# ZhangLearning/llm-message-queue

Hardware: AMD Instinct MI355X
Metric: requests/sec + p99 enqueue->dispatch latency, 4-tier mix at 1/2/4/8 backends (higher is better)
Workload: dtype bf16

## Files before the change

csrc/kernels/gemm_kernels.h:

```cpp
#pragma once

#include <hip/hip_runtime.h>
#include <stdint.h>

#include <type_traits>

#include "fp8_decode.h"
#include "sample_noise.h"

namespace llmq {

typedef __attribute__((ext_vector_type(8))) short gm_bf16x8;
typedef __attribute__((ext_vector_type(4))) float gm_f32x4;
typedef __attribute__((ext_vector_type(4))) unsigned int gm_u32x4;

constexpr int GM_BM = 256, GM_BN = 256, GM_BK = 64, GM_THREADS = 512;
constexpr int GM_HALF_BYTES = 128 * GM_BK * 2;
constexpr int GM_BUF_BYTES = 4 * GM_HALF_BYTES;
constexpr int GM_LDS_BYTES = 2 * GM_BUF_BYTES;
constexpr int GM_GROUP_M = 8;

enum { GM_EPI_STORE = 0, GM_EPI_SWIGLU = 2, GM_EPI_ROPE = 3, GM_EPI_ARGMAX = 4, GM_EPI_RESID = 5,
       GM_EPI_RESID_LDS = 6, GM_EPI_RESID_PRE = 7, GM_EPI_RESID_RMS = 8, GM_EPI_SAMPLE = 9 };
constexpr int GM_LDS_SPARE = 32768;
template <int EPI>
constexpr int gm_lds_bytes() { return EPI == GM_EPI_RESID_PRE ? GM_LDS_BYTES + GM_LDS_SPARE : GM_LDS_BYTES; }

enum {
  GM_DIAG_NONE = 0,
  GM_DIAG_SKIP_A2 = 1,
  GM_DIAG_NO_LDS_READ = 2,
  GM_DIAG_NO_DMA = 3,
  GM_DIAG_CLOCK = 4,
  GM_DIAG_CLOCK_NO_DMA = 5,
  GM_DIAG_L2_PANELS = 6
};

struct GmSide {
  float* pv;
  int32_t* pi;
  union {
    float* rpart;
    const float* inv_temp;
  };
  union {
    int* rticket;
    const uint32_t* key;
  };
  float* rscale;
  float reps;
};

struct GmRope {
  const int32_t* pos;
  const int32_t* slot;
  const float* cos_t;
  const float* sin_t;
  uint16_t* q;
  uint16_t* kc;
  uint16_t* vc;
  int Hq, Hkv, max_ctx, n_slots;
};
enum { GM_A0 = 0, GM_A1 = 1, GM_B0 = 2, GM_B1 = 3 };

__device__ __forceinline__ uint16_t gm_f2bf(float f) {
  uint32_t u = __float_as_uint(f);
  u += 0x7fffu + ((u >> 16) & 1u);
  return (uint16_t)(u >> 16);
}

__device__ __forceinline__ void gm_load_row_scales(const float* __restrict__ rs, int row0, int fq,
                                                   gm_f32x4 (&sc)[2][4]) {
  if (rs) {
#pragma unroll
    for (int mh = 0; mh < 2; ++mh)
#pragma unroll
      for (int m = 0; m < 4; ++m)
        sc[mh][m] = *reinterpret_cast<const gm_f32x4*>(rs + row0 + mh * 64 + m * 16 + fq * 4);
  } else {
#pragma unroll
    for (int mh = 0; mh < 2; ++mh)
#pragma unroll
      for (int m = 0; m < 4; ++m) sc[mh][m] = gm_f32x4{1.f, 1.f, 1.f, 1.f};
  }
}

#define GM_CPOL_SC1 16

struct GmSplit {
  int full;
  float* ws;
  int* cnt;
};

typedef __attribute__((address_space(3))) void* gm_lds_ptr;
typedef gm_f32x4 gm_acc_t[2][4][2][2];

__device__ __forceinline__ void gm_stage(__amdgpu_buffer_rsrc_t rs, uint32_t v0, uint32_t v1, uint32_t soff,
                                         uint8_t* smem, uint32_t dst0, uint32_t dst1) {
  __builtin_amdgcn_raw_ptr_buffer_load_lds(rs, (gm_lds_ptr)(smem + dst0), 16, v0, soff, 0, 0);
  __builtin_amdgcn_raw_ptr_buffer_load_lds(rs, (gm_lds_ptr)(smem + dst1), 16, v1, soff, 0, 0);
}

#define GM_LGKM(N) asm volatile("s_waitcnt lgkmcnt(" #N ")" ::: "memory")
#define GM_VMCNT(N) asm volatile("s_waitcnt vmcnt(%0)" ::"n"(N) : "memory")
#define GM_FENCE() __builtin_amdgcn_sched_barrier(0)
#define GM_BARRIER()                  \
  do {                                \
    GM_FENCE();                       \
    __builtin_amdgcn_s_barrier();     \
    GM_FENCE();                       \
  } while (0)

typedef __attribute__((ext_vector_type(2))) unsigned int gf_u32x2;
template <int OFF>
__device__ __forceinline__ gf_u32x2 gf_lds_read_b64(uint32_t addr) {
  gf_u32x2 r;
  asm volatile("ds_read_b64 %0, %1 offset:%2" : "=v"(r) : "v"(addr), "n"(OFF) : "memory");
  return r;
}

template <int PER>
__device__ __forceinline__ int gm_xcd_run_start(int b, int count) {
  const int n = PER * count;
  const int xcd = b & 7, q8 = n >> 3, r8 = n & 7;
  return xcd < r8 ? xcd * (q8 + 1) : r8 * (q8 + 1) + (xcd - r8) * q8;
}

struct GmTile {
  int tm, tn;
  int pid;
  int khalf;
};

__device__ __forceinline__ GmTile gm_tile_coords(int bid, int tiles_m, int tiles_n, int nwg, int full,
                                                 int group_m) {
  GmTile t;
  t.khalf = -1;
  if (bid < full) {
    t.pid = gm_xcd_run_start<1>(bid, full) + (bid >> 3);
  } else {
    const int b = bid - full;
    const int j = gm_xcd_run_start<2>(b, nwg - full) + (b >> 3);
    t.pid = full + (j >> 1);
    t.khalf = j & 1;
  }
  const int group = t.pid / (group_m * tiles_n);
  const int first_m = group * group_m;
  const int gsize = min(tiles_m - first_m, group_m);
  t.tm = first_m + (t.pid % (group_m * tiles_n)) % gsize;
  t.tn = (t.pid % (group_m * tiles_n)) / gsize;
  return t;
}

__device__ __forceinline__ bool gm_split_join(uint8_t* __restrict__ smem, gm_acc_t& acc, const GmSplit& sp,
                                              int tix) {
  const int tid = threadIdx.x;
  int* cnt = sp.cnt + 2 * tix;
  if (tid == 0) *reinterpret_cast<int*>(smem) =
      __hip_atomic_fetch_add(cnt, 1, __ATOMIC_RELAXED, __HIP_MEMORY_SCOPE_AGENT);
  __syncthreads();
  const int ticket = *reinterpret_cast<volatile int*>(smem);
  __syncthreads();
  float* slab = sp.ws + (size_t)tix * GM_THREADS * 128;
  const __amdgpu_buffer_rsrc_t srs = __builtin_amdgcn_make_buffer_rsrc(slab, 0, GM_THREADS * 32 * 16, 0x00020000);
  if (ticket == 0) {
#pragma unroll
    for (int a = 0; a < 2; ++a)
#pragma unroll
      for (int b = 0; b < 4; ++b)
#pragma unroll
        for (int c = 0; c < 2; ++c)
#pragma unroll
          for (int d = 0; d < 2; ++d)
          {
            const int i = ((a * 4 + b) * 4 + c * 2 + d) * GM_THREADS + tid;
            __builtin_amdgcn_raw_buffer_store_b128(__builtin_bit_cast(gm_u32x4, acc[a][b][c][d]), srs, i * 16,
                                                   0, GM_CPOL_SC1);
          }
    GM_VMCNT(0);
    __syncthreads();
    if (tid == 0) __hip_atomic_store(cnt + 1, 1, __ATOMIC_RELAXED, __HIP_MEMORY_SCOPE_AGENT);
    return true;
  }
  if (tid == 0) {
    for (int spin = 0; spin < (1 << 24); ++spin) {
      if (__hip_atomic_load(cnt + 1, __ATOMIC_RELAXED, __HIP_MEMORY_SCOPE_AGENT)) break;
      __builtin_amdgcn_s_sleep(2);
    }
    GM_VMCNT(0);
    __hip_atomic_store(cnt, 0, __ATOMIC_RELAXED, __HIP_MEMORY_SCOPE_AGENT);
    __hip_atomic_store(cnt + 1, 0, __ATOMIC_RELAXED, __HIP_MEMORY_SCOPE_AGENT);
  }
  __syncthreads();
#pragma unroll
  for (int a = 0; a < 2; ++a)
#pragma unroll
    for (int b = 0; b < 4; ++b)
#pragma unroll
      for (int c = 0; c < 2; ++c)
#pragma unroll
        for (int d = 0; d < 2; ++d)
        {
          const int i = ((a * 4 + b) * 4 + c * 2 + d) * GM_THREADS + tid;
          acc[a][b][c][d] += __builtin_bit_cast(gm_f32x4, __builtin_amdgcn_raw_buffer_load_b128(
                                 srs, i * 16, 0, GM_CPOL_SC1));
        }
  return false;
}


template <int EPI, int DIAG, bool FP8 = false>
__device__ __forceinline__ void gemm_tile(
    uint8_t* __restrict__ smem, const uint16_t* __restrict__ A, const void* __restrict__ W,
    const float* __restrict__ cs, uint16_t* __restrict__ C, int M, int N, int K, int group_m,
    const float* __restrict__ rs, const GmRope& rp, const GmSplit& sp, const GmSide& am, const int bid) {
  static_assert(!FP8 || (DIAG == GM_DIAG_NONE &&
                         (EPI == GM_EPI_STORE || EPI == GM_EPI_SWIGLU || EPI == GM_EPI_RESID_LDS)),
                "the FP8 form: STORE, SWIGLU and RESID_LDS, no diagnostics");
  constexpr int kBHalf = 128 * GM_BK * (FP8 ? 1 : 2);
  constexpr int kBuf = 2 * GM_HALF_BYTES + 2 * kBHalf;
  static_assert(2 * kBuf <= GM_LDS_BYTES, "operand buffers inside the launch's LDS");
  constexpr bool kStamp = DIAG == GM_DIAG_CLOCK || DIAG == GM_DIAG_CLOCK_NO_DMA;
  const int tiles_m = (M + GM_BM - 1) / GM_BM;
  const int tiles_n = N / GM_BN;
  const int nwg = tiles_m * tiles_n;
  const int full = sp.ws ? sp.full : nwg;
  const GmTile tile = gm_tile_coords(bid, tiles_m, tiles_n, nwg, full, group_m);
  const int pid = tile.pid, khalf = tile.khalf, tm = tile.tm, tn = tile.tn;

  const int tid = threadIdx.x;
  const int lane = tid & 63;
  const int w = __builtin_amdgcn_readfirstlane(tid >> 6);
  uint64_t st_t0 = 0, st_r0 = 0;
  if constexpr (kStamp) {
    st_t0 = __builtin_amdgcn_s_memtime();
    st_r0 = __builtin_amdgcn_s_memrealtime();
  }
  const int wr = w >> 2, wc = w & 3;

  const int srow = w * 8 + (lane >> 3);
  const int schunk = (lane & 7) ^ ((srow >> 1) & 7);
  const int brow = w * 16 + (lane >> 2);
  const int bchunk = (lane & 3) ^ ((brow >> 2) & 3);
  const __amdgpu_buffer_rsrc_t rsa = __builtin_amdgcn_make_buffer_rsrc((void*)A, 0, M * K * 2, 0x00020000);
  const __amdgpu_buffer_rsrc_t rsw =
      __builtin_amdgcn_make_buffer_rsrc((void*)W, 0, N * K * (FP8 ? 1 : 2), 0x00020000);
  uint32_t va[2][2], vb[2][FP8 ? 1 : 2];
  const int ltm = DIAG == GM_DIAG_L2_PANELS ? 0 : tm, ltn = DIAG == GM_DIAG_L2_PANELS ? 0 : tn;
#pragma unroll
  for (int h = 0; h < 2; ++h) {
#pragma unroll
    for (int i = 0; i < 2; ++i) {
      int row = ltm * GM_BM + i * 128 + h * 64 + srow;
      row = row < M ? row : M - 1;
      va[h][i] = (uint32_t)row * (uint32_t)K * 2u + (uint32_t)schunk * 16u;
      if constexpr (!FP8) {
        const int col = ltn * GM_BN + (2 * i + (w >> 2)) * 64 + h * 32 + (w & 3) * 8 + (lane >> 3);
        vb[h][i] = (uint32_t)col * (uint32_t)K * 2u + (uint32_t)schunk * 16u;
      }
    }
    if constexpr (FP8) {
      const int col = ltn * GM_BN + (brow >> 5) * 64 + h * 32 + (brow & 31);
      vb[h][0] = (uint32_t)col * (uint32_t)K + (uint32_t)bchunk * 16u;
    }
  }
  const uint32_t dst_i0 = (uint32_t)(w * 8) * 128u;
  const uint32_t dst_i1 = (uint32_t)(64 + w * 8) * 128u;
  const uint32_t dst_b = (uint32_t)(w * 16) * 64u;

  const uint32_t sbase = (uint32_t)(uintptr_t)(__attribute__((address_space(3))) uint8_t*)smem;
  const int fr = lane & 15, fq = lane >> 4;
  uint32_t aoff[2][2], boff[2][2];
#pragma unroll
  for (int kk = 0; kk < 2; ++kk) {
    const int c = fq + 4 * kk;
    aoff[0][kk] = (uint32_t)(wr * 64 + fr) * 128u + (uint32_t)((c ^ ((fr >> 1) & 7)) * 16);
    if constexpr (FP8)
      boff[0][kk] = (uint32_t)(2 * GM_HALF_BYTES) + (uint32_t)(wc * 32 + fr) * 64u +
                    (uint32_t)(((c >> 1) ^ ((fr >> 2) & 3)) * 16 + (c & 1) * 8);
    else
      boff[0][kk] = (uint32_t)(wc * 32 + fr) * 128u + (uint32_t)((c ^ ((fr >> 1) & 7)) * 16) + 2 * GM_HALF_BYTES;
    aoff[1][kk] = aoff[0][kk] + kBuf;
    boff[1][kk] = boff[0][kk] + kBuf;
  }

  gm_acc_t acc;
#pragma unroll
  for (int a = 0; a < 2; ++a)
#pragma unroll
    for (int b = 0; b < 4; ++b)
#pragma unroll
      for (int c = 0; c < 2; ++c)
#pragma unroll
        for (int d = 0; d < 2; ++d) acc[a][b][c][d] = gm_f32x4{0.f, 0.f, 0.f, 0.f};

  gm_bf16x8 af[4][2];
  using gm_bfrag = std::conditional_t<FP8, gf_u32x2, gm_bf16x8>;
  gm_bfrag bfr[2][2][2];
  gm_bfrag b0y[2][2];
  const int nt = khalf < 0 ? K / GM_BK : K / GM_BK / 2;
  const int kt0 = khalf > 0 ? nt : 0;

#define GM_STAGE(BUF, HALF, KT)                                                               \
  do {                                                                                        \
    if constexpr (FP8 && (HALF) >= 2) {                                                       \
      __builtin_amdgcn_raw_ptr_buffer_load_lds(                                               \
          rsw, (gm_lds_ptr)(smem + (uint32_t)(BUF) * kBuf + 2 * GM_HALF_BYTES + (uint32_t)((HALF)-2) * kBHalf + dst_b), \
          16, vb[(HALF)-2][0], (uint32_t)((KT) + kt0) * GM_BK, 0, 0);                         \
    } else {                                                                                  \
      const uint32_t _ko = (uint32_t)((KT) + kt0) * (GM_BK * 2);                              \
      const uint32_t _b = (uint32_t)(BUF) * kBuf + (uint32_t)(HALF) * GM_HALF_BYTES;          \
      if constexpr ((HALF) < 2)                                                               \
        gm_stage(rsa, va[(HALF)][0], va[(HALF)][1], _ko, smem, _b + dst_i0, _b + dst_i1);     \
      else                                                                                    \
        gm_stage(rsw, vb[(HALF)-2][0], vb[(HALF)-2][1], _ko, smem, _b + dst_i0, _b + dst_i1); \
    }                                                                                         \
  } while (0)

#define GM_READ_A(BUF, MH)                                                                     \
  do {                                                                                         \
    _Pragma("unroll") for (int m = 0; m < 4; ++m)                                              \
      _Pragma("unroll") for (int kk = 0; kk < 2; ++kk)                                         \
        af[m][kk] = *reinterpret_cast<const gm_bf16x8*>(smem + aoff[BUF][kk] + (MH) * GM_HALF_BYTES + m * 2048); \
  } while (0)

#define GM_READ_B_INTO(BUF, NH, DST)                                                           \
  do {                                                                                         \
    if constexpr (FP8) {                                                                       \
      _Pragma("unroll") for (int kk = 0; kk < 2; ++kk) {                                       \
        DST[0][kk] = gf_lds_read_b64<(NH) * kBHalf>(sbase + boff[BUF][kk]);                    \
        DST[1][kk] = gf_lds_read_b64<(NH) * kBHalf + 1024>(sbase + boff[BUF][kk]);             \
      }                                                                                        \
    } else {                                                                                   \
      _Pragma("unroll") for (int n = 0; n < 2; ++n)                                            \
        _Pragma("unroll") for (int kk = 0; kk < 2; ++kk)                                       \
          DST[n][kk] = *reinterpret_cast<const gm_bf16x8*>(smem + boff[BUF][kk] + (NH) * kBHalf + n * 2048); \
    }                                                                                          \
  } while (0)
#define GM_READ_B(BUF, NH) GM_READ_B_INTO(BUF, NH, bfr[NH])
#define GM_READ_B0_INTO(BUF, DST) GM_READ_B_INTO(BUF, 0, DST)

#define GM_MFMA_WITH(MH, NH, BREG)                                                             \
  do {                                                                                         \
    _Pragma("unroll") for (int kk = 0; kk < 2; ++kk) {                                         \
      gm_bf16x8 _b[2];                                                                         \
      _Pragma("unroll") for (int n = 0; n < 2; ++n) {                                          \
        if constexpr (FP8) _b[n] = sk_fp8x8_bf16(BREG[n][kk].x, BREG[n][kk].y);                \
        else _b[n] = BREG[n][kk];                                                              \
      }                                                                                        \
      _Pragma("unroll") for (int m = 0; m < 4; ++m)                                            \
        _Pragma("unroll") for (int n = 0; n < 2; ++n)                                          \
          acc[MH][m][NH][n] = __builtin_amdgcn_mfma_f32_16x16x32_bf16(af[m][kk], _b[n],        \
                                                                      acc[MH][m][NH][n], 0, 0, 0); \
    }                                                                                          \
  } while (0)

#define GM_PHASE_END(MH, NH, BREG)   \
  do {                               \
    GM_BARRIER();                    \
    GM_LGKM(0);                      \
    if constexpr (FP8) GM_FENCE();   \
    GM_MFMA_WITH(MH, NH, BREG);      \
    GM_BARRIER();                    \
  } while (0)

  constexpr int kDmaA = 2, kDmaB = FP8 ? 1 : 2;
  constexpr int kFlyA = 2 * kDmaA + kDmaB, kFlyB = kDmaA + 2 * kDmaB;

  if (wr == 1) __builtin_amdgcn_s_setprio(1);
  if constexpr (EPI == GM_EPI_RESID_PRE) {
    const int col0p = tn * GM_BN + wc * 64, row0p = tm * GM_BM + wr * 128;
    const __amdgpu_buffer_rsrc_t rsp =
        __builtin_amdgcn_make_buffer_rsrc((void*)C, 0, (uint32_t)M * (uint32_t)N * 2u, 0x00020000);
#pragma unroll
    for (int i = 0; i < 4; ++i) {
      const int r = i * 8 + (lane >> 3), c = lane & 7;
      const uint32_t vo = ((uint32_t)(row0p + r) * (uint32_t)N + (uint32_t)(col0p + c * 8)) * 2u;
      __builtin_amdgcn_raw_ptr_buffer_load_lds(rsp, (gm_lds_ptr)(smem + GM_LDS_BYTES + w * 4096 + i * 1024), 16,
                                               vo, 0, 0, 0);
    }
  }
  GM_STAGE(0, GM_B0, 0);
  GM_STAGE(0, GM_A0, 0);
  GM_STAGE(0, GM_B1, 0);
  GM_STAGE(0, GM_A1, 0);
  GM_STAGE(1, GM_B0, 1);
  GM_STAGE(1, GM_A0, 1);
  GM_STAGE(1, GM_B1, 1);
  GM_VMCNT(kFlyB);
  GM_BARRIER();
  GM_READ_B0_INTO(0, bfr[0]);
  if constexpr (DIAG >= GM_DIAG_SKIP_A2 && DIAG <= GM_DIAG_NO_DMA) {
    GM_READ_A(0, 0);
    GM_READ_B(0, 1);
    GM_READ_B0_INTO(1, b0y);
  }
  if (wr == 1) GM_BARRIER();

  int t = 0;
  constexpr bool kRdA = DIAG != GM_DIAG_NO_LDS_READ;
  constexpr bool kRdA2 = DIAG != GM_DIAG_SKIP_A2 && DIAG != GM_DIAG_NO_LDS_READ;
  constexpr bool kRdB = DIAG != GM_DIAG_NO_LDS_READ;
  constexpr bool kDma = DIAG != GM_DIAG_NO_DMA && DIAG != GM_DIAG_CLOCK_NO_DMA;
#define GM_D_READ_A(ON, B, H) do { if constexpr (ON) GM_READ_A(B, H); } while (0)
#define GM_D_READ_B(B, H) do { if constexpr (kRdB) GM_READ_B(B, H); } while (0)
#define GM_D_READ_B0(B, D) do { if constexpr (kRdB) GM_READ_B0_INTO(B, D); } while (0)
#define GM_D_STAGE(B, H, K) do { if constexpr (kDma) GM_STAGE(B, H, K); } while (0)
  for (; t < nt - 2; t += 2) {
    {
      GM_D_READ_A(kRdA, 0, 0); GM_D_STAGE(1, GM_A1, t + 1); GM_VMCNT(kFlyA); GM_PHASE_END(0, 0, bfr[0]);
      GM_D_READ_B(0, 1); GM_D_STAGE(0, GM_B0, t + 2); GM_VMCNT(kFlyB); GM_PHASE_END(0, 1, bfr[1]);
      GM_D_READ_A(kRdA2, 0, 1); GM_D_STAGE(0, GM_A0, t + 2); GM_VMCNT(kFlyA); GM_PHASE_END(1, 1, bfr[1]);
      GM_D_READ_B0(1, b0y); GM_D_STAGE(0, GM_B1, t + 2); GM_VMCNT(kFlyB); GM_PHASE_END(1, 0, bfr[0]);
      GM_D_READ_A(kRdA, 1, 0); GM_D_STAGE(0, GM_A1, t + 2); GM_VMCNT(kFlyA); GM_PHASE_END(0, 0, b0y);
      GM_D_READ_B(1, 1); GM_D_STAGE(1, GM_B0, t + 3); GM_VMCNT(kFlyB); GM_PHASE_END(0, 1, bfr[1]);
      GM_D_READ_A(kRdA2, 1, 1); GM_D_STAGE(1, GM_A0, t + 3); GM_VMCNT(kFlyA); GM_PHASE_END(1, 1, bfr[1]);
      GM_D_READ_B0(0, bfr[0]); GM_D_STAGE(1, GM_B1, t + 3); GM_VMCNT(kFlyB); GM_PHASE_END(1, 0, b0y);
    }
  }
  {
      GM_READ_A(0, 0); GM_STAGE(1, GM_A1, t + 1); GM_VMCNT(kFlyA); GM_PHASE_END(0, 0, bfr[0]);
      GM_READ_B(0, 1); GM_VMCNT(kDmaA + kDmaB); GM_PHASE_END(0, 1, bfr[1]);
      GM_READ_A(0, 1); GM_VMCNT(kDmaA); GM_PHASE_END(1, 1, bfr[1]);
      GM_READ_B0_INTO(1, b0y); GM_VMCNT(0); GM_PHASE_END(1, 0, bfr[0]);
      GM_READ_A(1, 0); GM_PHASE_END(0, 0, b0y);
      GM_READ_B(1, 1); GM_PHASE_END(0, 1, bfr[1]);
      GM_READ_A(1, 1); GM_PHASE_END(1, 1, bfr[1]);
      GM_PHASE_END(1, 0, b0y);
  }
  __builtin_amdgcn_s_setprio(0);
  if (wr == 0) GM_BARRIER();
#undef GM_D_READ_A
#undef GM_D_READ_B
#undef GM_D_READ_B0
#undef GM_D_STAGE
#undef GM_PHASE_END
#undef GM_MFMA_WITH
#undef GM_READ_B0_INTO
#undef GM_READ_B
#undef GM_READ_B_INTO
#undef GM_READ_A
#undef GM_STAGE

  if (khalf >= 0 && gm_split_join(smem, acc, sp, pid - full)) return;

  if constexpr (FP8) {
    const float* csp = cs + tn * GM_BN + wc * 64 + fr;
#pragma unroll
    for (int nh = 0; nh < 2; ++nh)
#pragma unroll
      for (int n = 0; n < 2; ++n) {
        const float s = csp[nh * 32 + n * 16];
#pragma unroll
        for (int mh = 0; mh < 2; ++mh)
#pragma unroll
          for (int m = 0; m < 4; ++m) acc[mh][m][nh][n] *= s;
      }
  }

  const int row0 = tm * GM_BM + wr * 128;
  if constexpr (EPI == GM_EPI_ARGMAX || EPI == GM_EPI_SAMPLE) {
    if constexpr (EPI == GM_EPI_SAMPLE) {
      const uint32_t col = (uint32_t)(tn * GM_BN + wc * 64 + fr);
#pragma unroll
      for (int mh = 0; mh < 2; ++mh)
#pragma unroll
        for (int m = 0; m < 4; ++m) {
          const int r4 = row0 + mh * 64 + m * 16 + fq * 4;
          const gm_f32x4 it = *reinterpret_cast<const gm_f32x4*>(am.inv_temp + r4);
          const gm_u32x4 ka = *reinterpret_cast<const gm_u32x4*>(am.key + 2 * r4);
          const gm_u32x4 kb = *reinterpret_cast<const gm_u32x4*>(am.key + 2 * r4 + 4);
#pragma unroll
          for (int j = 0; j < 4; ++j) {
            const uint32_t k0 = j < 2 ? ka[2 * j] : kb[2 * j - 4];
            const uint32_t k1 = j < 2 ? ka[2 * j + 1] : kb[2 * j - 3];
            if (it[j] != 0.f) {
#pragma unroll
              for (int nh = 0; nh < 2; ++nh)
#pragma unroll
                for (int n = 0; n < 2; ++n)
                  acc[mh][m][nh][n][j] = acc[mh][m][nh][n][j] * it[j] + sn_gumbel(k0, k1, col + nh * 32 + n * 16);
            }
          }
        }
    }
    float* lv = reinterpret_cast<float*>(smem);
    int* lc = reinterpret_cast<int*>(smem + GM_BM * 4 * 4);
#pragma unroll
    for (int mh = 0; mh < 2; ++mh)
#pragma unroll
      for (int m = 0; m < 4; ++m)
#pragma unroll
        for (int j = 0; j < 4; ++j) {
          float v = acc[mh][m][0][0][j];
          int c = fr;
#pragma unroll
          for (int nh = 0; nh < 2; ++nh)
#pragma unroll
            for (int n = 0; n < 2; ++n) {
              const float x = acc[mh][m][nh][n][j];
              if (x > v) { v = x; c = nh * 32 + n * 16 + fr; }
            }
#pragma unroll
          for (int off = 1; off < 16; off <<= 1) {
            const float ov = __shfl_xor(v, off, 64);
            const int oc = __shfl_xor(c, off, 64);
            if (ov > v || (ov == v && oc < c)) { v = ov; c = oc; }
          }
          if (fr == 0) {
            const int r = wr * 128 + mh * 64 + m * 16 + fq * 4 + j;
            lv[r * 4 + wc] = v;
            lc[r * 4 + wc] = wc * 64 + c;
          }
        }
    __syncthreads();
    if (tid < GM_BM) {
      const int grow = tm * GM_BM + tid;
      float v = lv[tid * 4];
      int c = lc[tid * 4];
#pragma unroll
      for (int k = 1; k < 4; ++k)
        if (lv[tid * 4 + k] > v) { v = lv[tid * 4 + k]; c = lc[tid * 4 + k]; }
      if (grow < M) {
        am.pv[(int64_t)grow * tiles_n + tn] = v;
        am.pi[(int64_t)grow * tiles_n + tn] = tn * GM_BN + c;
      }
    }
  } else if constexpr (EPI == GM_EPI_RESID) {
    float* o = reinterpret_cast<float*>(smem + w * (32 * 68 * 4));
    const int col0 = tn * GM_BN + wc * 64;
    uint2 cres[2][2][8];
#pragma unroll
    for (int mh = 0; mh < 2; ++mh)
#pragma unroll
      for (int mp = 0; mp < 2; ++mp)
#pragma unroll
        for (int it = 0; it < 8; ++it) {
          const int qd = it * 64 + lane;
          const int grow = row0 + mh * 64 + mp * 32 + (qd >> 4);
          cres[mh][mp][it] = grow < M ? *reinterpret_cast<const uint2*>(C + (int64_t)grow * N + col0 + (qd & 15) * 4)
                                      : make_uint2(0u, 0u);
        }
#pragma unroll
    for (int mh = 0; mh < 2; ++mh)
#pragma unroll
      for (int mp = 0; mp < 2; ++mp) {
#pragma unroll
        for (int mm = 0; mm < 2; ++mm)
#pragma unroll
          for (int nh = 0; nh < 2; ++nh)
#pragma unroll
            for (int n = 0; n < 2; ++n)
#pragma unroll
              for (int j = 0; j < 4; ++j)
                o[(mm * 16 + fq * 4 + j) * 68 + nh * 32 + n * 16 + fr] = acc[mh][mp * 2 + mm][nh][n][j];
        GM_LGKM(0);
        __builtin_amdgcn_wave_barrier();
#pragma unroll
        for (int it = 0; it < 8; ++it) {
          const int qd = it * 64 + lane;
          const int r = qd >> 4, c4 = qd & 15;
          const int grow = row0 + mh * 64 + mp * 32 + r;
          const gm_f32x4 v = *reinterpret_cast<const gm_f32x4*>(o + r * 68 + c4 * 4);
          if (grow < M) {
            uint2* cp = reinterpret_cast<uint2*>(C + (int64_t)grow * N + col0 + c4 * 4);
            const uint2 cr = cres[mh][mp][it];
            const float r0 = __uint_as_float(cr.x << 16) + v[0], r1 = __uint_as_float(cr.x & 0xffff0000u) + v[1];
            const float r2 = __uint_as_float(cr.y << 16) + v[2], r3 = __uint_as_float(cr.y & 0xffff0000u) + v[3];
            *cp = make_uint2((uint32_t)gm_f2bf(r0) | ((uint32_t)gm_f2bf(r1) << 16),
                             (uint32_t)gm_f2bf(r2) | ((uint32_t)gm_f2bf(r3) << 16));
          }
        }
        GM_LGKM(0);
        __builtin_amdgcn_wave_barrier();
      }
  } else if constexpr (EPI == GM_EPI_RESID_LDS || EPI == GM_EPI_RESID_PRE || EPI == GM_EPI_RESID_RMS) {
    constexpr int kPre = EPI == GM_EPI_RESID_PRE ? 4 : 0;
    uint8_t* cw = smem + w * 16384;
    uint8_t* cpre = smem + GM_LDS_BYTES + w * 4096;
    auto rowp = [&](int r) -> uint8_t* { return (kPre && r < 32) ? cpre + r * 128 : cw + r * 128; };
    const int col0 = tn * GM_BN + wc * 64;
    const __amdgpu_buffer_rsrc_t rsc =
        __builtin_amdgcn_make_buffer_rsrc((void*)C, 0, (uint32_t)M * (uint32_t)N * 2u, 0x00020000);
#pragma unroll
    for (int i = kPre; i < 16; ++i) {
      const int r = i * 8 + (lane >> 3), c = lane & 7;
      const uint32_t vo = ((uint32_t)(row0 + r) * (uint32_t)N + (uint32_t)(col0 + c * 8)) * 2u;
      __builtin_amdgcn_raw_ptr_buffer_load_lds(rsc, (gm_lds_ptr)(cw + i * 1024), 16, vo, 0, 0, 0);
    }
    GM_VMCNT(0);
    __builtin_amdgcn_wave_barrier();
#pragma unroll
    for (int mh = 0; mh < 2; ++mh)
#pragma unroll
      for (int m = 0; m < 4; ++m)
#pragma unroll
        for (int nh = 0; nh < 2; ++nh)
#pragma unroll
          for (int n = 0; n < 2; ++n)
#pragma unroll
            for (int j = 0; j < 4; ++j) {
              const int r = mh * 64 + m * 16 + fq * 4 + j;
              uint16_t* e = reinterpret_cast<uint16_t*>(rowp(r) + (nh * 32 + n * 16 + fr) * 2);
              *e = gm_f2bf(__uint_as_float((uint32_t)*e << 16) + acc[mh][m][nh][n][j]);
            }
    GM_LGKM(0);
    __builtin_amdgcn_wave_barrier();
    constexpr bool rms = EPI == GM_EPI_RESID_RMS;
    float ssq[16];
#pragma unroll
    for (int it = 0; it < 16; ++it) {
      const int qd = it * 64 + lane;
      const int r = qd >> 3, cb = qd & 7;
      const int grow = row0 + r;
      const gm_u32x4 v = *reinterpret_cast<const gm_u32x4*>(rowp(r) + cb * 16);
      if (grow < M) *reinterpret_cast<gm_u32x4*>(C + (int64_t)grow * N + col0 + cb * 8) = v;
      if constexpr (rms) {
        float q = 0.f;
#pragma unroll
        for (int e = 0; e < 4; ++e) {
          const float lo = __uint_as_float(v[e] << 16), hi = __uint_as_float(v[e] & 0xFFFF0000u);
          q += lo * lo + hi * hi;
        }
        ssq[it] = q;
      }
    }
    if constexpr (rms) {
#pragma unroll
      for (int it = 0; it < 16; ++it) {
        float q = ssq[it];
        q += __shfl_xor(q, 1, 64);
        q += __shfl_xor(q, 2, 64);
        q += __shfl_xor(q, 4, 64);
        ssq[it] = q;
      }
      GM_LGKM(0);
      __builtin_amdgcn_wave_barrier();
      float* wp = reinterpret_cast<float*>(cw);
      if ((lane & 7) == 0) {
#pragma unroll
        for (int it = 0; it < 16; ++it) wp[it * 8 + (lane >> 3)] = ssq[it];
      }
      __syncthreads();
      const int tiles_n_ = N / GM_BN;
      if (tid < 256) {
        const int hw = tid >> 7, rr = tid & 127;
        float sum = 0.f;
#pragma unroll
        for (int c = 0; c < 4; ++c) sum += reinterpret_cast<const float*>(smem + (hw * 4 + c) * 16384)[rr];
        const __amdgpu_buffer_rsrc_t prs = __builtin_amdgcn_make_buffer_rsrc(
            am.rpart + (size_t)(tm * tiles_n_ + tn) * 256, 0, 256 * 4, 0x00020000);
        __builtin_amdgcn_raw_buffer_store_b32(__float_as_uint(sum), prs, tid * 4, 0, GM_CPOL_SC1);
      }
      GM_VMCNT(0);
      __syncthreads();
      if (tid == 0)
        *reinterpret_cast<int*>(smem) = __hip_atomic_fetch_add(am.rticket + tm, 1, __ATOMIC_RELAXED,
                                                               __HIP_MEMORY_SCOPE_AGENT);
      __syncthreads();
      const int done = *reinterpret_cast<volatile int*>(smem);
      if (done == tiles_n_ - 1 && tid < 256) {
        float sum = 0.f;
        for (int t2 = 0; t2 < tiles_n_; ++t2) {
          const __amdgpu_buffer_rsrc_t prs = __builtin_amdgcn_make_buffer_rsrc(
              am.rpart + (size_t)(tm * tiles_n_ + t2) * 256, 0, 256 * 4, 0x00020000);
          sum += __uint_as_float(__builtin_amdgcn_raw_buffer_load_b32(prs, tid * 4, 0, GM_CPOL_SC1));
        }
        am.rscale[tm * 256 + tid] = rsqrtf(sum / (float)N + am.reps);
        if (tid == 0) __hip_atomic_store(am.rticket + tm, 0, __ATOMIC_RELAXED, __HIP_MEMORY_SCOPE_AGENT);
      }
    }
  } else if constexpr (EPI == GM_EPI_SWIGLU) {
    uint16_t* o = reinterpret_cast<uint16_t*>(smem + w * 8192);
    gm_f32x4 sc[2][4];
    gm_load_row_scales(rs, row0, fq, sc);
#pragma unroll
    for (int mh = 0; mh < 2; ++mh)
#pragma unroll
      for (int m = 0; m < 4; ++m)
#pragma unroll
        for (int n = 0; n < 2; ++n)
#pragma unroll
          for (int j = 0; j < 4; ++j) {
            const float g = acc[mh][m][0][n][j] * sc[mh][m][j];
            const float u = acc[mh][m][1][n][j] * sc[mh][m][j];
            const float s = g / (1.0f + __expf(-g));
            o[(mh * 64 + m * 16 + fq * 4 + j) * 32 + n * 16 + fr] = gm_f2bf(s * u);
          }
    GM_LGKM(0);
    __builtin_amdgcn_wave_barrier();
    const int F = N >> 1;
    const int col0 = tn * (GM_BN / 2) + wc * 32;
#pragma unroll
    for (int it = 0; it < 8; ++it) {
      const int qd = it * 64 + lane;
      const int r = qd >> 2, cb = qd & 3;
      const int grow = row0 + r;
      const gm_u32x4 v = *reinterpret_cast<const gm_u32x4*>(smem + w * 8192 + r * 64 + cb * 16);
      if (grow < M) *reinterpret_cast<gm_u32x4*>(C + (int64_t)grow * F + col0 + cb * 8) = v;
    }
  } else {
    uint16_t* o = reinterpret_cast<uint16_t*>(smem + w * 16384);
    gm_f32x4 sc[2][4];
    gm_load_row_scales(rs, row0, fq, sc);
#pragma unroll
    for (int mh = 0; mh < 2; ++mh)
#pragma unroll
      for (int m = 0; m < 4; ++m)
#pragma unroll
        for (int nh = 0; nh < 2; ++nh)
#pragma unroll
          for (int n = 0; n < 2; ++n)
#pragma unroll
            for (int j = 0; j < 4; ++j)
              o[(mh * 64 + m * 16 + fq * 4 + j) * 64 + nh * 32 + n * 16 + fr] =
                  gm_f2bf(acc[mh][m][nh][n][j] * sc[mh][m][j]);
    if constexpr (EPI == GM_EPI_STORE) {
      GM_LGKM(0);
      __builtin_amdgcn_wave_barrier();
      const int col0 = tn * GM_BN + wc * 64;
#pragma unroll
      for (int it = 0; it < 16; ++it) {
        const int qd = it * 64 + lane;
        const int r = qd >> 3, cb = qd & 7;
        const int grow = row0 + r;
        const gm_u32x4 v = *reinterpret_cast<const gm_u32x4*>(smem + w * 16384 + r * 128 + cb * 16);
        if (grow < M) *reinterpret_cast<gm_u32x4*>(C + (int64_t)grow * N + col0 + cb * 8) = v;
      }
    } else {
      __syncthreads();
      auto at = [&](int r, int c) -> const uint8_t* {
        return smem + ((r >> 7) * 4 + (c >> 6)) * 16384 + (r & 127) * 128 + (c & 63) * 2;
      };
      const int nq = rp.Hq / 2, nk = rp.Hkv / 2;
      if (tn < nq + nk) {
        const int hh = (tid >> 3) & 1, j = tid & 7, r0 = tid >> 4;
        int pk[8], sk[8];
#pragma unroll
        for (int k = 0; k < 8; ++k) {
          const int grow = min(tm * GM_BM + r0 + 32 * k, M - 1);
          pk[k] = rp.pos[grow];
          sk[k] = rp.slot[grow];
        }
        float4 c0[8], c1[8], s0[8], s1[8];
#pragma unroll
        for (int k = 0; k < 8; ++k) {
          const int64_t o = (int64_t)min(max(pk[k], 0), rp.max_ctx - 1) * 64 + 8 * j;
          c0[k] = *reinterpret_cast<const float4*>(rp.cos_t + o);
          c1[k] = *reinterpret_cast<const float4*>(rp.cos_t + o + 4);
          s0[k] = *reinterpret_cast<const float4*>(rp.sin_t + o);
          s1[k] = *reinterpret_cast<const float4*>(rp.sin_t + o + 4);
        }
#pragma unroll
        for (int k = 0; k < 8; ++k) {
          const int r = r0 + 32 * k;
          const int grow = tm * GM_BM + r;
          const int p = pk[k], sl = sk[k];
          if (grow >= M || (unsigned)sl >= (unsigned)rp.n_slots || (unsigned)p >= (unsigned)rp.max_ctx) continue;
          const gm_u32x4 lo = *reinterpret_cast<const gm_u32x4*>(at(r, hh * 128 + 8 * j));
          const gm_u32x4 hi = *reinterpret_cast<const gm_u32x4*>(at(r, hh * 128 + 64 + 8 * j));
          const float cc[8] = {c0[k].x, c0[k].y, c0[k].z, c0[k].w, c1[k].x, c1[k].y, c1[k].z, c1[k].w};
          const float ss[8] = {s0[k].x, s0[k].y, s0[k].z, s0[k].w, s1[k].x, s1[k].y, s1[k].z, s1[k].w};
          gm_u32x4 olo, ohi;
#pragma unroll
          for (int e = 0; e < 4; ++e) {
            const float a0 = __uint_as_float(lo[e] << 16), a1 = __uint_as_float(lo[e] & 0xffff0000u);
            const float b0 = __uint_as_float(hi[e] << 16), b1 = __uint_as_float(hi[e] & 0xffff0000u);
            const float c_0 = cc[2 * e], c_1 = cc[2 * e + 1], s_0 = ss[2 * e], s_1 = ss[2 * e + 1];
            olo[e] = (uint32_t)gm_f2bf(a0 * c_0 - b0 * s_0) | ((uint32_t)gm_f2bf(a1 * c_1 - b1 * s_1) << 16);
            ohi[e] = (uint32_t)gm_f2bf(b0 * c_0 + a0 * s_0) | ((uint32_t)gm_f2bf(b1 * c_1 + a1 * s_1) << 16);
          }
          uint16_t* dst;
          if (tn < nq) {
            dst = rp.q + (int64_t)grow * rp.Hq * 128 + (2 * tn + hh) * 128;
          } else {
            const int kvh = 2 * (tn - nq) + hh;
            dst = rp.kc + (((int64_t)sl * rp.Hkv + kvh) * rp.max_ctx + p) * 128;
          }
          *reinterpret_cast<gm_u32x4*>(dst + 8 * j) = olo;
          *reinterpret_cast<gm_u32x4*>(dst + 64 + 8 * j) = ohi;
        }
      } else {
        const int hh = (tid >> 4) & 1, cb = tid & 15, r0 = tid >> 5;
        int pk[16], sk[16];
#pragma unroll
        for (int k = 0; k < 16; ++k) {
          const int grow = min(tm * GM_BM + r0 + 16 * k, M - 1);
          pk[k] = rp.pos[grow];
          sk[k] = rp.slot[grow];
        }
        const int kvh = 2 * (tn - nq - nk) + hh;
#pragma unroll
        for (int k = 0; k < 16; ++k) {
          const int r = r0 + 16 * k;
          const int grow = tm * GM_BM + r;
          const int p = pk[k], sl = sk[k];
          if (grow >= M || (unsigned)sl >= (unsigned)rp.n_slots || (unsigned)p >= (unsigned)rp.max_ctx) continue;
          uint16_t* dst = rp.vc + (((int64_t)sl * rp.Hkv + kvh) * rp.max_ctx + p) * 128;
          *reinterpret_cast<gm_u32x4*>(dst + 8 * cb) = *reinterpret_cast<const gm_u32x4*>(at(r, hh * 128 + 8 * cb));
        }
      }
    }
  }
  if constexpr (kStamp) {
    const uint64_t st_t1 = __builtin_amdgcn_s_memtime(), st_r1 = __builtin_amdgcn_s_memrealtime();
    if (tid == 0 && am.pv != nullptr) {
      uint64_t* dbg = reinterpret_cast<uint64_t*>(am.pv) + (size_t)bid * 4;
      dbg[0] = st_t0;
      dbg[1] = st_t1;
      dbg[2] = st_r0;
      dbg[3] = st_r1;
    }
  }
}

template <int EPI, int DIAG = GM_DIAG_NONE>
__global__ __launch_bounds__(GM_THREADS) void gemm_bf16_kernel(
    const uint16_t* __restrict__ A, const uint16_t* __restrict__ W, uint16_t* __restrict__ C,
    int M, int N, int K, int group_m, const float* __restrict__ rs, const GmRope rp, const GmSplit sp,
    const GmSide am) {
  extern __shared__ __align__(16) uint8_t smem[];
  gemm_tile<EPI, DIAG>(smem, A, W, nullptr, C, M, N, K, group_m, rs, rp, sp, am, (int)blockIdx.x);
}

template <int EPI>
__global__ __launch_bounds__(GM_THREADS) void gemm_fp8w_kernel(
    const uint16_t* __restrict__ A, const uint8_t* __restrict__ Wq, const float* __restrict__ cs,
    uint16_t* __restrict__ C, int M, int N, int K, int group_m, const float* __restrict__ rs, const GmSplit sp) {
  extern __shared__ __align__(16) uint8_t smem[];
  gemm_tile<EPI, GM_DIAG_NONE, true>(smem, A, Wq, cs, C, M, N, K, group_m, rs, GmRope{}, sp, GmSide{},
                                     (int)blockIdx.x);
}

__global__ __launch_bounds__(256) void gemm_argmax_reduce_kernel(const float* __restrict__ pv,
                                                                 const int32_t* __restrict__ pi, int M, int tiles,
                                                                 int32_t* __restrict__ out) {
  const int row = blockIdx.x * 4 + (threadIdx.x >> 6);
  const int lane = threadIdx.x & 63;
  if (row >= M) return;
  float v = -__builtin_inff();
  int c = 0x7fffffff;
  for (int t = lane; t < tiles; t += 64) {
    const float x = pv[(int64_t)row * tiles + t];
    if (x > v) { v = x; c = pi[(int64_t)row * tiles + t]; }
  }
#pragma unroll
  for (int off = 1; off < 64; off <<= 1) {
    const float ov = __shfl_xor(v, off, 64);
    const int oc = __shfl_xor(c, off, 64);
    if (ov > v || (ov == v && oc < c)) { v = ov; c = oc; }
  }
  if (lane == 0) out[row] = c == 0x7fffffff ? 0 : c;
}

__global__ __launch_bounds__(256) void sample_bits_kernel(const uint32_t* __restrict__ keys, uint32_t n0, int count,
                                                          uint32_t* __restrict__ out) {
  const int i = blockIdx.x * 256 + threadIdx.x;
  const int k = blockIdx.y;
  if (i < count) out[(int64_t)k * count + i] = sn_bits(keys[2 * k], keys[2 * k + 1], n0 + (uint32_t)i);
}

#undef GM_LGKM
#undef GM_VMCNT
#undef GM_BARRIER
#undef GM_FENCE

}
```

Baseline: 5418.

## Transpose SwiGLU accumulator layout and vectorize swizzled epilogue stores

For the SwiGLU epilogue, the MFMA operands are swapped so each lane's accumulator holds consecutive output columns instead of rows. This lets the epilogue pack pairs of bf16 values and write 8-byte chunks into an XOR-swizzled LDS staging area instead of scalar 2-byte stores. It also uses exp2 with a pre-multiplied constant for the sigmoid and adjusts the FP8 column-scale load to the new layout. Row scales become per-lane scalars. The aim is to cut LDS store count and bank conflicts in the epilogue, at the risk of layout mistakes in the swizzle and scale indexing.

```diff
diff --git a/csrc/kernels/gemm_kernels.h b/csrc/kernels/gemm_kernels.h
--- a/csrc/kernels/gemm_kernels.h
+++ b/csrc/kernels/gemm_kernels.h
@@ -13,6 +13,8 @@
 typedef __attribute__((ext_vector_type(8))) short gm_bf16x8;
 typedef __attribute__((ext_vector_type(4))) float gm_f32x4;
 typedef __attribute__((ext_vector_type(4))) unsigned int gm_u32x4;
+typedef __attribute__((ext_vector_type(2))) float gm_f32x2;
+typedef __attribute__((ext_vector_type(2))) __bf16 gm_bf16x2;
 
 constexpr int GM_BM = 256, GM_BN = 256, GM_BK = 64, GM_THREADS = 512;
 constexpr int GM_HALF_BYTES = 128 * GM_BK * 2;
@@ -222,6 +224,7 @@
   constexpr int kBuf = 2 * GM_HALF_BYTES + 2 * kBHalf;
   static_assert(2 * kBuf <= GM_LDS_BYTES, "operand buffers inside the launch's LDS");
   constexpr bool kStamp = DIAG == GM_DIAG_CLOCK || DIAG == GM_DIAG_CLOCK_NO_DMA;
+  constexpr bool kAccT = EPI == GM_EPI_SWIGLU;
   const int tiles_m = (M + GM_BM - 1) / GM_BM;
   const int tiles_n = N / GM_BN;
   const int nwg = tiles_m * tiles_n;
@@ -350,9 +353,14 @@
         else _b[n] = BREG[n][kk];                                                              \
       }                                                                                        \
       _Pragma("unroll") for (int m = 0; m < 4; ++m)                                            \
-        _Pragma("unroll") for (int n = 0; n < 2; ++n)                                          \
-          acc[MH][m][NH][n] = __builtin_amdgcn_mfma_f32_16x16x32_bf16(af[m][kk], _b[n],        \
-                                                                      acc[MH][m][NH][n], 0, 0, 0); \
+        _Pragma("unroll") for (int n = 0; n < 2; ++n) {                                        \
+          if constexpr (kAccT)                                                                 \
+            acc[MH][m][NH][n] = __builtin_amdgcn_mfma_f32_16x16x32_bf16(_b[n], af[m][kk],      \
+                                                                        acc[MH][m][NH][n], 0, 0, 0); \
+          else                                                                                 \
+            acc[MH][m][NH][n] = __builtin_amdgcn_mfma_f32_16x16x32_bf16(af[m][kk], _b[n],      \
+                                                                        acc[MH][m][NH][n], 0, 0, 0); \
+        }                                                                                      \
     }                                                                                          \
   } while (0)
 
@@ -445,7 +453,19 @@
 
   if (khalf >= 0 && gm_split_join(smem, acc, sp, pid - full)) return;
 
-  if constexpr (FP8) {
+  if constexpr (FP8 && kAccT) {
+    const float* csp = cs + tn * GM_BN + wc * 64 + fq * 4;
+#pragma unroll
+    for (int nh = 0; nh < 2; ++nh)
+#pragma unroll
+      for (int n = 0; n < 2; ++n) {
+        const gm_f32x4 s = *reinterpret_cast<const gm_f32x4*>(csp + nh * 32 + n * 16);
+#pragma unroll
+        for (int mh = 0; mh < 2; ++mh)
+#pragma unroll
+          for (int m = 0; m < 4; ++m) acc[mh][m][nh][n] *= s;
+      }
+  } else if constexpr (FP8) {
     const float* csp = cs + tn * GM_BN + wc * 64 + fr;
 #pragma unroll
     for (int nh = 0; nh < 2; ++nh)
@@ -672,22 +692,43 @@
       }
     }
   } else if constexpr (EPI == GM_EPI_SWIGLU) {
-    uint16_t* o = reinterpret_cast<uint16_t*>(smem + w * 8192);
-    gm_f32x4 sc[2][4];
-    gm_load_row_scales(rs, row0, fq, sc);
+    float sc[2][4];
+    if (rs) {
+#pragma unroll
+      for (int mh = 0; mh < 2; ++mh)
+#pragma unroll
+        for (int m = 0; m < 4; ++m) sc[mh][m] = rs[row0 + mh * 64 + m * 16 + fr];
+    } else {
+#pragma unroll
+      for (int mh = 0; mh < 2; ++mh)
+#pragma unroll
+        for (int m = 0; m < 4; ++m) sc[mh][m] = 1.f;
+    }
+    const int wsw = ((fr >> 1) & 3) << 1;
+    uint8_t* ow[2];
+    ow[0] = smem + w * 8192 + fr * 64 + ((fq ^ wsw) << 3);
+    ow[1] = smem + w * 8192 + fr * 64 + (((4 + fq) ^ wsw) << 3);
+    constexpr float kNegLog2e = -0x1.715476p+0f;
 #pragma unroll
     for (int mh = 0; mh < 2; ++mh)
 #pragma unroll
       for (int m = 0; m < 4; ++m)
 #pragma unroll
-        for (int n = 0; n < 2; ++n)
-#pragma unroll
-          for (int j = 0; j < 4; ++j) {
-            const float g = acc[mh][m][0][n][j] * sc[mh][m][j];
-            const float u = acc[mh][m][1][n][j] * sc[mh][m][j];
-            const float s = g / (1.0f + __expf(-g));
-            o[(mh * 64 + m * 16 + fq * 4 + j) * 32 + n * 16 + fr] = gm_f2bf(s * u);
+        for (int n = 0; n < 2; ++n) {
+          const gm_f32x4 g4 = acc[mh][m][0][n] * sc[mh][m];
+          const gm_f32x4 u4 = acc[mh][m][1][n] * sc[mh][m];
+          gf_u32x2 pk;
+#pragma unroll
+          for (int p = 0; p < 2; ++p) {
+            const gm_f32x2 g = {g4[2 * p], g4[2 * p + 1]}, u = {u4[2 * p], u4[2 * p + 1]};
+            const gm_f32x2 t = g * kNegLog2e;
+            const gm_f32x2 e = {__builtin_amdgcn_exp2f(t.x), __builtin_amdgcn_exp2f(t.y)};
+            const gm_f32x2 d = 1.0f + e;
+            const gm_f32x2 s = {g.x / d.x, g.y / d.y};
+            pk[p] = __builtin_bit_cast(uint32_t, __builtin_convertvector(s * u, gm_bf16x2));
           }
+          *reinterpret_cast<gf_u32x2*>(ow[n] + mh * 4096 + m * 1024) = pk;
+        }
     GM_LGKM(0);
     __builtin_amdgcn_wave_barrier();
     const int F = N >> 1;
@@ -697,7 +738,8 @@
       const int qd = it * 64 + lane;
       const int r = qd >> 2, cb = qd & 3;
       const int grow = row0 + r;
-      const gm_u32x4 v = *reinterpret_cast<const gm_u32x4*>(smem + w * 8192 + r * 64 + cb * 16);
+      const gm_u32x4 v =
+          *reinterpret_cast<const gm_u32x4*>(smem + w * 8192 + r * 64 + ((cb ^ ((r >> 1) & 3)) << 4));
       if (grow < M) *reinterpret_cast<gm_u32x4*>(C + (int64_t)grow * F + col0 + cb * 8) = v;
     }
   } else {
```

Result: no change. 5427, median of 6 (+0.2%).
